# Charrrrrlie/X-as-Supervision

Hardware: AMD Instinct MI355X
Metric: images/sec HM36_Multi_SurS1 256px bs32 (full disc+gen training step) (higher is better)
Workload: dtype f32 (f16x3 split: every fp32 operand as two fp16 pieces, three products; f32 accumulate); 1 GPU; HM36_Multi_SurS1; batch_per_gpu=32, cameras=4, image=256x256, parallelism=dp1, ranks=1, precision=f16x3, dedupe=False, full=False

## Files before the change

include/xas_hip.h:

```cpp
#ifndef XAS_HIP_H
#define XAS_HIP_H

#include <stddef.h>
#include <stdint.h>

#ifdef __cplusplus
extern "C" {
#endif

const char* xas_last_error(void);
enum {
  XAS_TUNE_WGRAD_SPLIT_XCD = 1,
  XAS_TUNE_PLAIN_KLOOP = 32,
  XAS_TUNE_GLOBAL_LOAD = 64,
  XAS_TUNE_WGRAD_GLOBAL_LOAD = 128,
  XAS_TUNE_WGRAD_ALT_ORDER = 8192,
  XAS_TUNE_WGRAD_PLAIN_KLOOP = 524288,
  XAS_TUNE_SLAB_SHIFT = 15,
  XAS_TUNE_SLAB_MASK = 3,
  XAS_TUNE_SLAB_512 = 32768,
  XAS_TUNE_SLAB_128 = 65536,
  XAS_TUNE_SLAB_64 = 98304,
  XAS_TUNE_COL_REDUCE_LEAN = 262144,
  XAS_TUNE_GENERAL_KERNELS = 1 << 22,
// ... 164 lines not shown
int xas_mask_blur_threshold(const uint8_t* mask, int B, int P, uint8_t* out, void* stream);
int xas_patch_finish(const uint8_t* img_bgr, const uint8_t* mask, const float* color_scale, const float* mean3,
                     const float* std3, int rm_bg, int B, int P, float* out_img, float* out_mask, void* stream);
size_t xas_geodesic_workspace_bytes(int B, int P);
int xas_geodesic_weight(const float* mask, const int* centers, const float* params5, int B, int P, float* out,
                        int* center_out, void* workspace, void* stream);
int xas_geodesic_weight_multi(const float* mask, const int* centers, int num_centers, int order, const float* params5, int B, int P,
                              float* out, int* center_out, void* workspace, void* stream);

int xas_loss_nblk(long n);
int xas_mask_loss_fwd(const float* m, const float* gt, const float* weight, long n, int mode,
                      float* partial, float* out, void* stream);
int xas_mask_loss_bwd(const float* m, const float* gt, const float* weight, long n, int mode,
                      const float* out, const float* grad_scalar, float* dm, void* stream);

int xas_pose_loss_fwd(const float* pred, const float* gt, int B, int Hy, int K, int kind, float w0, float w1,
                      float w2, float* out, void* stream);
int xas_pose_loss_bwd(const float* pred, const float* gt, int B, int Hy, int K, int kind, float w0, float w1,
                      float w2, const float* out, const float* grad_scalar, float* grad_pred, float* grad_aux,
                      void* stream);
int xas_lsgan_fwd(const float* logits, int B, int Hy, float target, float* out, int* idx, void* stream);
int xas_lsgan_bwd(const float* logits, int B, int Hy, float target, const int* idx, const float* grad_scalar,
                  float* grad_logits, void* stream);

int xas_graph_aggregate(const float* x, const float* adj, int B, int N, int C, float* y, void* stream);
size_t xas_gln_workspace_floats(long n, int groups, int C);
int xas_gln_fwd(const float* x, const float* gamma, const float* beta, const float* residual,
                long rows, int C, int groups, float eps, float* y, float* stats, float* workspace,
                void* stream);
int xas_gln_bwd(const float* x, const float* beta, const float* dy, const float* gamma,
                const float* stats, long rows, int C, int groups, float eps, float* dx, float* dgamma,
                float* dbeta, float* workspace, void* stream);

int xas_smpl_lbs_fwd(const float* pose , const float* betas ,
                     const float* v_template , const float* shapedirs ,
                     const float* posedirs , const float* j_regressor ,
                     const float* weights , const int* parents , int B, int V,
                     int center_idx, float* verts , float* joints ,
                     float* workspace , void* stream);

size_t xas_smpl_lbs_bwd_workspace_floats(int B, int V);
int xas_smpl_lbs_bwd(const float* pose, const float* betas, const float* v_template, const float* shapedirs,
                     const float* posedirs, const float* j_regressor, const float* weights, const int* parents, int B,
                     int V, int center_idx, const float* fwd_workspace, const float* d_verts, const float* d_joints,
                     float* d_pose, float* d_betas, float* workspace, void* stream);

int xas_adam_step(float* p, const float* g, float* m, float* v, long n, float lr, float beta1,
                  float beta2, float eps, int step, void* stream);


#define XAS_EVAL_CONFIDENT 1
#define XAS_EVAL_SWITCH_ALL 2
#define XAS_EVAL_GT_NORMALISED 4
int xas_eval_select(const float* kps, const float* joints, const int* perm, int B, int Hy, int K, int C,
                    float image_size, int flags, float* sel3d, float* sel2d, float* err2d,
                    unsigned char* swapped, void* stream);

int xas_projection_matrix(const float* k_mat, const float* rot_world, const float* trans_world, int B, float* P,
                          void* stream);

int xas_triangulate_dlt(const float* points, const float* P, int B, int V, int K, float* out, void* stream);

int xas_pose_metrics(const float* pred, const float* gt, const unsigned char* mask, int N, int K, float in_div,
                     int pck_align, float pck_threshold, float* err, float* aligned, float* pck, int* auc_hits,
                     void* stream);

// ... 5 lines not shown
```

x-as-supervision_amd/modules/discriminator.py:

```python
import math

import torch
import torch.nn as nn

from modules.gcn import GCN_SAGE_residual, GCN_residual, GCN_simple
from xas_amd import layers as L


class FFNHeader(nn.Module):
    def __init__(self, in_channels, hidden_channels, p_dropout=0.2):
        super().__init__()
        self.layer1 = L.Linear(in_channels, hidden_channels)
        self.layer2 = L.Linear(hidden_channels, 1)
        self.p = p_dropout
        self.drop_mask = None

    def forward(self, x):
        h = torch.relu(self.layer1(x))
        if self.training and self.p > 0:
            keep = self.drop_mask if self.drop_mask is not None else (torch.rand_like(h) >= self.p).to(h.dtype)
            h = h * keep / (1.0 - self.p)
        return self.layer2(h)


class GCNDiscriminator_base(nn.Module):
    def __init__(self, cfg):
        super().__init__()
        self.input_dim = cfg['input_dim']
        self.hidden_dim = cfg['hidden_dim']
        self.output_dim = cfg['output_dim']
        self.disc_sup_dim = cfg['disc_sup_dim']
        self.num_nodes = cfg['num_node']
        self.use_self_loop = cfg['use_self_loop']
        self.input_layer = nn.Identity()
        self.gcn = nn.Identity()
        self.header = L.Linear(self.output_dim * self.num_nodes, 1)
        self.parent_ids, self.child_ids = None, None
        self._graph_key, self._graph = None, None
# ... 55 lines not shown
            self.num_layers = cfg['num_layers']
            self.gcn = nn.Sequential(
                GCN_simple(self.input_dim, self.hidden_dim, self_loop=sl),
                *[GCN_residual(self.hidden_dim, self.hidden_dim, self.hidden_dim, self_loop=sl, use_bn=cfg['use_bn'])
                  for _ in range(self.num_layers)],
                GCN_simple(self.hidden_dim, self.output_dim, self_loop=sl))
        else:
            raise NotImplementedError
        self.input_layer = L.Linear(self.disc_sup_dim, self.input_dim)

    def compute_graph_matrix(self, keypoints):
        B = keypoints.shape[0]
        pidx, cidx = self._bone_index(keypoints.device)
        diff = keypoints[:, pidx, :] - keypoints[:, cidx, :]
        inv = 1.0 / torch.sqrt(torch.sum(diff ** 2, dim=-1))
        n = self.num_nodes
        w = torch.eye(n, device=keypoints.device).repeat(B, 1, 1) if self.use_self_loop else \
            torch.zeros(B, n, n, device=keypoints.device)
        w = w.index_put((torch.arange(B, device=keypoints.device)[:, None], pidx[None, :], cidx[None, :]), inv)
        w = w.index_put((torch.arange(B, device=keypoints.device)[:, None], cidx[None, :], pidx[None, :]), inv)
        return w

    def forward(self, keypoints):
        B = keypoints.shape[0]
        adj = self.compute_graph_matrix(keypoints)
        x = self.input_layer(keypoints.reshape(B * self.num_nodes, -1))
        return self.header_forward(self.gcn((x, adj))[0], B)

    def forward_groups(self, inputs):
        return [self(x) for x in inputs]


def _stream(hidden, out, num_layers):
    return nn.Sequential(*[GCN_SAGE_residual(hidden, hidden, hidden) for _ in range(num_layers)],
                         GCN_SAGE_residual(hidden, -1, out, single_layer=True))


class GCNSAGEDiscriminator(GCNDiscriminator_base):
    def __init__(self, cfg):
        super().__init__(cfg)
        self.name = 'ResSAGEGCN'
        self.num_layers = cfg['num_layers']
        self.gcn = _stream(self.hidden_dim, self.output_dim, self.num_layers)
        self.use_pe = cfg['use_pe'] if 'use_pe' in cfg else False
        self.input_layer = L.Linear(self.disc_sup_dim * (2 if self.use_pe else 1), self.input_dim)

    def _forward(self, keypoints, groups=1):
        B = keypoints.shape[0]
        g = self.graph(B, keypoints.device) + (groups,)
        if self.use_pe:
            keypoints = torch.cat([keypoints, self.cal_positional_encoding(keypoints)], dim=-1)
        x = self.input_layer(keypoints.reshape(B * self.num_nodes, -1))
        return self.header_forward(self.gcn((x, g))[0], B)


class GCNDiscriminatorDecouple(GCNDiscriminator_base):
    def __init__(self, cfg):
        super().__init__(cfg)
        self.use_pe = cfg['use_pe'] if 'use_pe' in cfg else False
        cin = self.disc_sup_dim * (2 if self.use_pe else 1)
        self.joint_input_layer = L.Linear(cin, self.input_dim)
        self.bone_input_layer = L.Linear(cin, self.input_dim)
        self.name = 'ResGCNDecouple'
        self.num_layers = cfg['num_layers']
        self.joint_gcn = _stream(self.hidden_dim, self.output_dim, self.num_layers)
        self.bone_gcn = _stream(self.hidden_dim, self.output_dim, self.num_layers)
        self.header = FFNHeader(self.output_dim * self.num_nodes * 2, 512)

# ... 19 lines not shown
```

x-as-supervision_amd/modules/gcn.py:

```python
import torch
import torch.nn as nn

from xas_amd import layers as L
from xas_amd import ops_misc


def my_batched_dense_to_sparse(adj):
    if adj.dim() < 2 or adj.dim() > 3:
        raise ValueError(f"Dense adjacency matrix 'adj' must be two- or three-dimensional (got {adj.dim()} dimensions)")
    if adj.dim() == 2:
        idx = adj.nonzero().t()
        return idx, adj[idx[0], idx[1]]
    B, N, M = adj.shape
    flat = adj.reshape(B * N, M)
    idx = flat.nonzero().t().clone()
    vals = flat[idx[0], idx[1]]
    idx[1] += (idx[0] // N) * M
    return idx, vals


class SAGEConv(nn.Module):

    def __init__(self, cin, cout):
        super().__init__()
        self.lin_l = L.Linear(cin, cout, bias=True)
        self.lin_r = L.Linear(cin, cout, bias=False)

    def forward(self, x, graph):
        adj, adj_t, B, N = graph[:4]
        return self.lin_l(ops_misc.graph_aggregate(x, adj, adj_t, B, N)) + self.lin_r(x)


class GraphLayerNorm(nn.Module):
    def __init__(self, c, eps=1e-5):
        super().__init__()
        self.eps = eps
        self.weight = nn.Parameter(torch.ones(c))
        self.bias = nn.Parameter(torch.zeros(c))


class GCN_SAGE_residual(nn.Module):
    def __init__(self, input_dim, hidden_dim, output_dim, single_layer=False):
        super().__init__()
        self.single_layer = single_layer
        if single_layer:
            self.gc1 = SAGEConv(input_dim, output_dim)
            self.ln1 = GraphLayerNorm(output_dim)
            self.gc2 = nn.Identity()
        else:
            self.gc1 = SAGEConv(input_dim, hidden_dim)
            self.ln1 = GraphLayerNorm(hidden_dim)
            self.gc2 = SAGEConv(hidden_dim, output_dim)
            self.ln2 = GraphLayerNorm(output_dim)

    def forward(self, input):
        x, graph = input
        groups = graph[4] if len(graph) > 4 else 1
        y = ops_misc.graph_layernorm_relu(self.gc1(x, graph), self.ln1.weight, self.ln1.bias, None, self.ln1.eps, groups)
        if self.single_layer:
            return (y, graph)
        y = ops_misc.graph_layernorm_relu(self.gc2(y, graph), self.ln2.weight, self.ln2.bias, x, self.ln2.eps, groups)
        return (y, graph)


class GCNConv(nn.Module):

    def __init__(self, cin, cout, add_self_loops=True):
        super().__init__()
        self.lin = L.Linear(cin, cout, bias=False)
        self.bias = nn.Parameter(torch.zeros(cout))
        self.add_self_loops = add_self_loops

    def norm(self, adj):
        if self.add_self_loops:
            diag = adj.diagonal(dim1=1, dim2=2)
            adj = adj + torch.diag_embed((diag == 0).to(adj.dtype))
        deg = adj.sum(dim=1)
        dis = deg.pow(-0.5)
        dis = torch.where(torch.isinf(dis), torch.zeros_like(dis), dis)
        return dis.unsqueeze(2) * adj * dis.unsqueeze(1)

    def forward(self, x, adj):
        B, N = adj.shape[:2]
        xw = self.lin(x).view(B, N, -1)
        out = torch.bmm(self.norm(adj).transpose(1, 2), xw)
        return out.reshape(B * N, -1) + self.bias


class GCN_simple(nn.Module):
    def __init__(self, input_dim, output_dim, self_loop=False):
        super().__init__()
        self.gc = GCNConv(input_dim, output_dim, add_self_loops=self_loop)

    def forward(self, input):
        x, adj = input
# ... 31 lines not shown
```

x-as-supervision_amd/xas_amd/_lib.py:

```python
import ctypes
import os

import torch

_HERE = os.path.dirname(os.path.abspath(__file__))
LIB_PATH = os.environ.get('XAS_HIP_LIB') or os.path.join(_HERE, 'libxas_hip.so')
_lib = None
ABI_VERSION = 3

_T = {'p': ctypes.c_void_p, 'i': ctypes.c_int, 'l': ctypes.c_long, 'f': ctypes.c_float, 'u': ctypes.c_uint,
      'd': ctypes.c_double, 'z': ctypes.c_size_t}


class ConvShape(ctypes.Structure):
    _fields_ = [(n, ctypes.c_int) for n in ('N', 'Hi', 'Wi', 'Cin', 'Cout', 'R', 'S', 'stride', 'pad', 'Ho', 'Wo', 'mode')] + [
        ('grad_amax', ctypes.c_void_p),
        ('x_amax', ctypes.c_void_p)]


PREC_F32, PREC_BF16, PREC_BF16X6, PREC_F16X3 = 0, 1, 2, 3
PREC_NAMES = {'f32': PREC_F32, 'bf16': PREC_BF16, 'bf16x6': PREC_BF16X6, 'f16x3': PREC_F16X3}

TUNE_WGRAD_SPLIT_XCD = 1
TUNE_PLAIN_KLOOP, TUNE_GLOBAL_LOAD, TUNE_WGRAD_GLOBAL_LOAD = 32, 64, 128
# ... 55 lines not shown
    'xas_col_sum_acc': ('plippp', 'i'),
    'xas_bn_apply': ('ppppppfiliippp', 'i'),
    'xas_bn_apply_amax': ('ppppppfiliipppp', 'i'),
    'xas_abs_max': ('plpp', 'i'),
    'xas_bn_update_running': ('ppppfliip', 'i'),
    'xas_bn_bwd_reduce': ('pppppppfiliipppppp', 'i'),
    'xas_bn_bwd_apply': ('ppppppppfiliidpppp', 'i'),
    'xas_bn_bwd_apply_amax': ('ppppppppfiliidppppp', 'i'),
    'xas_maxpool3x3s2_fwd': ('piiiippp', 'i'),
    'xas_maxpool3x3s2_bwd': ('ppiiiipp', 'i'),
    'xas_upsample2x_fwd': ('piiiipp', 'i'),
    'xas_upsample2x_bwd': ('piiiipp', 'i'),
    'xas_sigmoid_fwd': ('plpp', 'i'),
    'xas_sigmoid_bwd': ('pplpp', 'i'),
    'xas_nchw_to_nhwc': ('piiiipp', 'i'),
    'xas_nhwc_to_nchw': ('piiiipp', 'i'),
    'xas_warp_affine_u8': ('ppppiiipp', 'i'),
    'xas_mask_blur_threshold': ('piipp', 'i'),
    'xas_patch_finish': ('pppppiiippp', 'i'),
    'xas_geodesic_workspace_bytes': ('ii', 'z'),
    'xas_geodesic_weight': ('pppiipppp', 'i'),
    'xas_geodesic_weight_multi': ('ppiipiipppp', 'i'),
    'xas_loss_nblk': ('l', 'i'),
    'xas_mask_loss_fwd': ('pppliPpp'.replace('P', 'p'), 'i'),
    'xas_mask_loss_bwd': ('pppliPppp'.replace('P', 'p'), 'i'),
    'xas_pose_loss_fwd': ('ppiiiifffpp', 'i'),
    'xas_pose_loss_bwd': ('ppiiiifffppppp', 'i'),
    'xas_lsgan_fwd': ('piifppp', 'i'),
    'xas_lsgan_bwd': ('piifpppp', 'i'),
    'xas_graph_aggregate': ('ppiiipp', 'i'),
    'xas_gln_workspace_floats': ('lii', 'z'),
    'xas_gln_fwd': ('ppppliifpppp', 'i'),
    'xas_gln_bwd': ('pppppliifppppp', 'i'),
    'xas_smpl_lbs_fwd': ('ppppppppiiipppp', 'i'),
    'xas_smpl_lbs_bwd_workspace_floats': ('ii', 'z'),
    'xas_smpl_lbs_bwd': ('ppppppppiiippppppp', 'i'),
    'xas_adam_step': ('pppplffffip', 'i'),
    'xas_eval_select': ('pppiiiifippppp', 'i'),
    'xas_projection_matrix': ('pppipp', 'i'),
    'xas_triangulate_dlt': ('ppiiipp', 'i'),
    'xas_pose_metrics': ('pppiififppppp', 'i'),
}


def load():
    global _lib
    if _lib is not None:
        return _lib
    if not os.path.exists(LIB_PATH):
        raise RuntimeError('libxas_hip.so is missing (%s): run `python __graft_entry__.py` to build the HIP '
                           'library; the MI355X path has no CPU fallback' % LIB_PATH)
    lib = ctypes.CDLL(LIB_PATH)
    lib.xas_abi_version.restype = ctypes.c_int
    lib.xas_abi_version.argtypes = []
    if lib.xas_abi_version() != ABI_VERSION:
        raise RuntimeError('%s speaks ABI version %d, this binding expects %d (include/xas_hip.h): rebuild it with '
                           '`python __graft_entry__.py`' % (LIB_PATH, lib.xas_abi_version(), ABI_VERSION))
    lib.xas_last_error.restype = ctypes.c_char_p
    lib.xas_last_error.argtypes = []
    _lib = lib
    mode = os.environ.get('XAS_PRECISION', '')
    if mode != '':
        lib.xas_set_precision.argtypes = [ctypes.c_int]
        lib.xas_set_precision.restype = ctypes.c_int
        if lib.xas_set_precision(int(mode)) != 0:
            raise RuntimeError('XAS_PRECISION=%s: %s' % (mode, lib.xas_last_error().decode()))
# ... 49 lines not shown
```

x-as-supervision_amd/xas_amd/ops_misc.py:

```python
import torch

from ._lib import call, ptr, query


class _MaskLoss(torch.autograd.Function):
    @staticmethod
    def forward(ctx, m, gt, weight, use_clip):
        m, gt = m.contiguous(), gt.contiguous()
        w = weight.contiguous() if weight is not None else None
        n = m.numel()
        mode = (1 if use_clip else 0) | (2 if w is not None else 0)
        partial = torch.empty(query('xas_loss_nblk', n) * 2, device=m.device, dtype=torch.float32)
        out = torch.empty(3, device=m.device, dtype=torch.float32)
        call('xas_mask_loss_fwd', ptr(m), ptr(gt), ptr(w), n, mode, ptr(partial), ptr(out))
        ctx.save_for_backward(m, gt, w if w is not None else m.new_empty(0), out)
        ctx.mode = mode
        return out[2]

    @staticmethod
    def backward(ctx, g):
        m, gt, w, out = ctx.saved_tensors
        dm = torch.empty_like(m)
        call('xas_mask_loss_bwd', ptr(m), ptr(gt), ptr(w) if ctx.mode & 2 else None, m.numel(), ctx.mode, ptr(out),
             ptr(g.contiguous().reshape(1)), ptr(dm))
        return dm, None, None, None


def mask_loss(mask, gt, weight=None, use_clip=False):
    return _MaskLoss.apply(mask, gt, weight, use_clip)


class _GraphAggregate(torch.autograd.Function):
    @staticmethod
    def forward(ctx, x, adj, adj_t, B, N):
# ... 21 lines not shown

class _GraphLayerNormRelu(torch.autograd.Function):
    @staticmethod
    def forward(ctx, x, gamma, beta, residual, eps, groups):
        x = x.contiguous()
        rows_all, C = x.shape
        rows = rows_all // groups
        y = torch.empty_like(x)
        stats = torch.empty(groups * 2, device=x.device, dtype=torch.float32)
        ws = torch.empty(query('xas_gln_workspace_floats', rows * C, groups, C), device=x.device, dtype=torch.float32)
        res = residual.contiguous() if residual is not None else None
        call('xas_gln_fwd', ptr(x), ptr(gamma), ptr(beta), ptr(res), rows, C, groups, float(eps), ptr(y), ptr(stats), ptr(ws))
        ctx.save_for_backward(x, gamma, beta, stats)
        ctx.cfg = (float(eps), residual is not None, groups, rows)
        return y

    @staticmethod
    def backward(ctx, dy):
        x, gamma, beta, stats = ctx.saved_tensors
        eps, has_res, groups, rows = ctx.cfg
        C = x.shape[1]
        dy = dy.contiguous()
        dx = torch.empty_like(x)
        dg = torch.empty_like(gamma)
        db = torch.empty_like(beta)
        ws = torch.empty(query('xas_gln_workspace_floats', rows * C, groups, C), device=x.device, dtype=torch.float32)
        call('xas_gln_bwd', ptr(x), ptr(beta), ptr(dy), ptr(gamma), ptr(stats), rows, C, groups, eps, ptr(dx), ptr(dg),
             ptr(db), ptr(ws))
        return dx, dg, db, (dy if has_res else None), None, None


def graph_layernorm_relu(x, gamma, beta, residual=None, eps=1e-5, groups=1):
    return _GraphLayerNormRelu.apply(x, gamma, beta, residual, eps, groups)


class _SmplLbs(torch.autograd.Function):

    @staticmethod
    def forward(ctx, pose, betas, v_template, shapedirs, posedirs, j_regressor, weights, parents, center_idx):
        B, V = pose.shape[0], v_template.shape[-2]
        dev = pose.device
        pose, betas = pose.contiguous(), betas.contiguous()
        bufs = tuple(t.contiguous() for t in (v_template, shapedirs, posedirs, j_regressor, weights))
        verts = torch.empty(B, V, 3, device=dev, dtype=torch.float32)
        joints = torch.empty(B, 24, 3, device=dev, dtype=torch.float32)
        ws = torch.empty(B * (72 + 24 * 16 + 207), device=dev, dtype=torch.float32)
        c = -1 if center_idx is None else int(center_idx)
        call('xas_smpl_lbs_fwd', ptr(pose), ptr(betas), *(ptr(t) for t in bufs), ptr(parents), B, V, c, ptr(verts),
             ptr(joints), ptr(ws))
        ctx.save_for_backward(pose, betas, *bufs, parents, ws)
        ctx.cfg = (B, V, c)
        return verts, joints

    @staticmethod
    def backward(ctx, d_verts, d_joints):
        pose, betas, vt, sd, pd, jr, w, parents, ws = ctx.saved_tensors
        B, V, c = ctx.cfg
        d_pose, d_betas = torch.empty_like(pose), torch.empty_like(betas)
        dv = d_verts.contiguous() if d_verts is not None else torch.zeros(B, V, 3, device=pose.device)
        dj = d_joints.contiguous() if d_joints is not None else None
        ws2 = torch.empty(query('xas_smpl_lbs_bwd_workspace_floats', B, V), device=pose.device, dtype=torch.float32)
        call('xas_smpl_lbs_bwd', ptr(pose), ptr(betas), ptr(vt), ptr(sd), ptr(pd), ptr(jr), ptr(w), ptr(parents), B, V, c,
             ptr(ws), ptr(dv), ptr(dj), ptr(d_pose), ptr(d_betas), ptr(ws2))
        return d_pose, d_betas, None, None, None, None, None, None, None


# ... 61 lines not shown
```

Before: 2078 images/s.

## Fuse GraphSAGE residual stack into tiled MFMA kernels with inline layernorm

Adds a fused HIP path for stacks of SAGEConv + graph layernorm + ReLU + residual layers in the discriminator. Each forward kernel applies the previous layer's layernorm and ReLU, does the adjacency aggregation in shared memory, and runs both linear projections with fp32 MFMA. It also emits per-tile partial statistics so the next layer can normalise without a separate pass. The backward pass has fused data and parameter-gradient kernels that write gradients straight into existing .grad buffers. This replaces many small launches and intermediate tensors, but adds a large amount of custom code and shape restrictions (C≤128, N≤18).

```diff
diff --git a/include/xas_hip.h b/include/xas_hip.h
--- a/include/xas_hip.h
+++ b/include/xas_hip.h
@@ -220,6 +220,28 @@
                 const float* stats, long rows, int C, int groups, float eps, float* dx, float* dgamma,
                 float* dbeta, float* workspace, void* stream);
 
+int xas_sage_tile_samples(void);
+int xas_sage_tiles(int B, int groups);
+int xas_sage_fwd(const float* zin, const float* part_in, const float* gamma, const float* beta,
+                 const float* res, float* h_out, float* stats_out, const float* adj, const float* wl,
+                 const float* bl, const float* wr, int B, int N, int C, int groups, float eps, float* z,
+                 float* part_out, void* stream);
+int xas_sage_ln_apply(const float* z, const float* part, const float* gamma, const float* beta,
+                      const float* res, int B, int N, int C, int groups, float eps, float* h,
+                      float* stats, void* stream);
+int xas_sage_ln_bwd_sums(const float* g, const float* z, const float* stats, const float* gamma,
+                         const float* beta, int B, int N, int C, int groups, float eps, float* psum,
+                         void* stream);
+int xas_sage_bwd_data(const float* g, const float* z, const float* stats, const float* psum,
+                      const float* gamma, const float* beta, const float* wl, const float* wr,
+                      const float* adj_t, const float* gres, const float* z_below,
+                      const float* stats_below, const float* gamma_below, const float* beta_below,
+                      int B, int N, int C, int groups, float eps, float eps_below, float* dz,
+                      float* g_below, float* psum_below, void* stream);
+int xas_sage_bwd_params(const float* dz, const float* h, const float* adj, const float* psum, int B,
+                        int N, int C, int groups, float* gwl, float* gbl, float* gwr, float* ggamma,
+                        float* gbeta, void* stream);
+
 int xas_smpl_lbs_fwd(const float* pose , const float* betas ,
                      const float* v_template , const float* shapedirs ,
                      const float* posedirs , const float* j_regressor ,
diff --git a/x-as-supervision_amd/csrc/gcn.hip b/x-as-supervision_amd/csrc/gcn.hip
--- /dev/null
+++ b/x-as-supervision_amd/csrc/gcn.hip
@@ -0,0 +1,562 @@
+#include "common.h"
+
+namespace xas {
+
+typedef float f32x16 __attribute__((ext_vector_type(16)));
+
+constexpr int kSageT = 3;
+constexpr int kSageMaxN = 18;
+constexpr int kSageMaxC = 128;
+constexpr int kSageRows = kSageT * kSageMaxN;
+constexpr int kSageLD = kSageMaxC + 4;
+
+__device__ __forceinline__ float gln_xhat(float x, float mean, float inv) { return __fmul_rn(__fsub_rn(x, mean), inv); }
+__device__ __forceinline__ float gln_pre(float xh, float g, float b) { return __fmaf_rn(xh, g, b); }
+
+struct SageTile {
+  int g, ti, R;
+  long row0;
+};
+__device__ __forceinline__ SageTile sage_tile(int B, int N, int tpg) {
+  SageTile t;
+  t.g = blockIdx.x / tpg;
+  t.ti = blockIdx.x % tpg;
+  const int s0 = t.ti * kSageT;
+  const int ns = (B - s0 < kSageT) ? B - s0 : kSageT;
+  t.R = ns * N;
+  t.row0 = ((long)t.g * B + s0) * N;
+  return t;
+}
+
+__device__ __forceinline__ void sage_group_stats(const float* __restrict__ part, int g, int tpg, float* out) {
+  const int lane = threadIdx.x & 63;
+  const float* pg = part + (size_t)g * tpg * 4;
+  const double P = (double)pg[0];
+  double a = 0.0, b = 0.0, n = 0.0;
+  for (int i = lane; i < tpg; i += 64) {
+    const double d = (double)pg[i * 4] - P, cnt = (double)pg[i * 4 + 1], s1 = (double)pg[i * 4 + 2], s2 = (double)pg[i * 4 + 3];
+    a += s1 + cnt * d;
+    b += s2 + 2.0 * d * s1 + cnt * d * d;
+    n += cnt;
+  }
+#pragma unroll
+  for (int o = 32; o > 0; o >>= 1) {
+    a += __shfl_xor(a, o, 64);
+    b += __shfl_xor(b, o, 64);
+    n += __shfl_xor(n, o, 64);
+  }
+  if (lane == 0) {
+    const double m = a / n;
+    double v = b / n - m * m;
+    if (v < 0.0) v = 0.0;
+    out[0] = (float)(P + m);
+    out[1] = (float)sqrt(v);
+  }
+}
+
+__device__ __forceinline__ f32x16 zero16() {
+  f32x16 v;
+#pragma unroll
+  for (int e = 0; e < 16; ++e) v[e] = 0.f;
+  return v;
+}
+
+__device__ __forceinline__ int mfma_row(int reg, int half) { return (reg & 3) + 8 * (reg >> 2) + 4 * half; }
+
+struct SageFwdArgs {
+  const float* zin;
+  const float* part_in;
+  const float* gamma;
+  const float* beta;
+  const float* res;
+  float* h_out;
+  float* stats_out;
+  const float* adj;
+  const float* wl;
+  const float* bl;
+  const float* wr;
+  float* z;
+  float* part_out;
+  int B, N, C, tpg;
+  float eps;
+};
+
+__global__ __launch_bounds__(256) void sage_fwd_kernel(SageFwdArgs a) {
+  __shared__ __attribute__((aligned(16))) float hs[kSageRows * kSageLD];
+  __shared__ __attribute__((aligned(16))) float ags[kSageRows * kSageLD];
+  __shared__ float adj_s[kSageMaxN * kSageMaxN];
+  __shared__ float st[2];
+  __shared__ float red[20];
+  __shared__ float s_piv;
+  const SageTile t = sage_tile(a.B, a.N, a.tpg);
+  const int C = a.C, N = a.N, R = t.R, C4 = C >> 2;
+  const int tid = threadIdx.x, lane = tid & 63, wave = tid >> 6;
+  for (int e = tid; e < N * N; e += 256) adj_s[e] = a.adj[e];
+  if (a.part_in && tid < 64) sage_group_stats(a.part_in, t.g, a.tpg, st);
+  __syncthreads();
+  float mean = 0.f, inv = 0.f;
+  if (a.part_in) {
+    mean = st[0];
+    inv = 1.f / (st[1] + a.eps);
+    if (t.ti == 0 && tid == 0) { a.stats_out[t.g * 2] = st[0]; a.stats_out[t.g * 2 + 1] = st[1]; }
+  }
+  for (int e = tid; e < R * C4; e += 256) {
+    const int r = e / C4, c = (e % C4) * 4;
+    const size_t off = (size_t)(t.row0 + r) * C + c;
+    float4 v = *reinterpret_cast<const float4*>(a.zin + off);
+    if (a.part_in) {
+      const float4 g4 = *reinterpret_cast<const float4*>(a.gamma + c), b4 = *reinterpret_cast<const float4*>(a.beta + c);
+      v.x = fmaxf(gln_pre(gln_xhat(v.x, mean, inv), g4.x, b4.x), 0.f);
+      v.y = fmaxf(gln_pre(gln_xhat(v.y, mean, inv), g4.y, b4.y), 0.f);
+      v.z = fmaxf(gln_pre(gln_xhat(v.z, mean, inv), g4.z, b4.z), 0.f);
+      v.w = fmaxf(gln_pre(gln_xhat(v.w, mean, inv), g4.w, b4.w), 0.f);
+      if (a.res) {
+        const float4 r4 = *reinterpret_cast<const float4*>(a.res + off);
+        v.x += r4.x; v.y += r4.y; v.z += r4.z; v.w += r4.w;
+      }
+      *reinterpret_cast<float4*>(a.h_out + off) = v;
+    }
+    *reinterpret_cast<float4*>(&hs[r * kSageLD + c]) = v;
+  }
+  __syncthreads();
+  for (int e = tid; e < R * C4; e += 256) {
+    const int r = e / C4, c = (e % C4) * 4;
+    const int node = r % N, sb = r - node;
+    float4 acc = make_float4(0.f, 0.f, 0.f, 0.f);
+    for (int j = 0; j < N; ++j) {
+      const float w = adj_s[node * N + j];
+      if (w != 0.f) {
+        const float4 x4 = *reinterpret_cast<const float4*>(&hs[(sb + j) * kSageLD + c]);
+        acc.x = fmaf(w, x4.x, acc.x); acc.y = fmaf(w, x4.y, acc.y); acc.z = fmaf(w, x4.z, acc.z); acc.w = fmaf(w, x4.w, acc.w);
+      }
+    }
+    *reinterpret_cast<float4*>(&ags[r * kSageLD + c]) = acc;
+  }
+  __syncthreads();
+  const int j = lane & 31, hh = lane >> 5, n0 = wave * 32;
+  const int nmb = (R + 31) >> 5;
+  f32x16 acc[2];
+  float sa = 0.f, sb2 = 0.f;
+  if (n0 < C) {
+    const float bias = a.bl[n0 + j];
+#pragma unroll
+    for (int e = 0; e < 16; ++e) { acc[0][e] = bias; acc[1][e] = bias; }
+    const int r0 = (j < R) ? j : R - 1, r1 = (32 + j < R) ? 32 + j : R - 1;
+#pragma unroll
+    for (int ph = 0; ph < 2; ++ph) {
+      const float* A = ph ? hs : ags;
+      const float* W = (ph ? a.wr : a.wl) + (size_t)(n0 + j) * C + 4 * hh;
+      const float* A0 = A + r0 * kSageLD + 4 * hh;
+      const float* A1 = A + r1 * kSageLD + 4 * hh;
+
+      for (int q = 0; q < C; q += 8) {
+        const float4 b4 = *reinterpret_cast<const float4*>(W + q);
+        const float4 a0 = *reinterpret_cast<const float4*>(A0 + q);
+        acc[0] = __builtin_amdgcn_mfma_f32_32x32x2f32(a0.x, b4.x, acc[0], 0, 0, 0);
+        acc[0] = __builtin_amdgcn_mfma_f32_32x32x2f32(a0.y, b4.y, acc[0], 0, 0, 0);
+        acc[0] = __builtin_amdgcn_mfma_f32_32x32x2f32(a0.z, b4.z, acc[0], 0, 0, 0);
+        acc[0] = __builtin_amdgcn_mfma_f32_32x32x2f32(a0.w, b4.w, acc[0], 0, 0, 0);
+        if (nmb > 1) {
+          const float4 a1 = *reinterpret_cast<const float4*>(A1 + q);
+          acc[1] = __builtin_amdgcn_mfma_f32_32x32x2f32(a1.x, b4.x, acc[1], 0, 0, 0);
+          acc[1] = __builtin_amdgcn_mfma_f32_32x32x2f32(a1.y, b4.y, acc[1], 0, 0, 0);
+          acc[1] = __builtin_amdgcn_mfma_f32_32x32x2f32(a1.z, b4.z, acc[1], 0, 0, 0);
+          acc[1] = __builtin_amdgcn_mfma_f32_32x32x2f32(a1.w, b4.w, acc[1], 0, 0, 0);
+        }
+      }
+    }
+    if (wave == 0 && lane == 0) s_piv = acc[0][0];
+  }
+  __syncthreads();
+  if (n0 < C) {
+    const float piv = s_piv;
+#pragma unroll
+    for (int mb = 0; mb < 2; ++mb) {
+#pragma unroll
+      for (int reg = 0; reg < 16; ++reg) {
+        const int row = mb * 32 + mfma_row(reg, hh);
+        if (row < R) {
+          const float v = acc[mb][reg];
+          a.z[(size_t)(t.row0 + row) * C + n0 + j] = v;
+          const float d = v - piv;
+          sa += d;
+          sb2 = fmaf(d, d, sb2);
+        }
+      }
+    }
+  }
+  sa = block_sum(sa, red);
+  sb2 = block_sum(sb2, red);
+  if (tid == 0) {
+    float* o = a.part_out + (size_t)blockIdx.x * 4;
+    o[0] = s_piv; o[1] = (float)(R * C); o[2] = sa; o[3] = sb2;
+  }
+}
+
+__global__ __launch_bounds__(256) void sage_ln_apply_kernel(const float* __restrict__ z, const float* __restrict__ part,
+                                                            const float* __restrict__ gamma, const float* __restrict__ beta,
+                                                            const float* __restrict__ res, int B, int N, int C, int tpg,
+                                                            float eps, float* __restrict__ h, float* __restrict__ stats) {
+  __shared__ float st[2];
+  const SageTile t = sage_tile(B, N, tpg);
+  const int tid = threadIdx.x, C4 = C >> 2;
+  if (tid < 64) sage_group_stats(part, t.g, tpg, st);
+  __syncthreads();
+  const float mean = st[0], inv = 1.f / (st[1] + eps);
+  if (t.ti == 0 && tid == 0) { stats[t.g * 2] = st[0]; stats[t.g * 2 + 1] = st[1]; }
+  for (int e = tid; e < t.R * C4; e += 256) {
+    const int r = e / C4, c = (e % C4) * 4;
+    const size_t off = (size_t)(t.row0 + r) * C + c;
+    float4 v = *reinterpret_cast<const float4*>(z + off);
+    const float4 g4 = *reinterpret_cast<const float4*>(gamma + c), b4 = *reinterpret_cast<const float4*>(beta + c);
+    v.x = fmaxf(gln_pre(gln_xhat(v.x, mean, inv), g4.x, b4.x), 0.f);
+    v.y = fmaxf(gln_pre(gln_xhat(v.y, mean, inv), g4.y, b4.y), 0.f);
+    v.z = fmaxf(gln_pre(gln_xhat(v.z, mean, inv), g4.z, b4.z), 0.f);
+    v.w = fmaxf(gln_pre(gln_xhat(v.w, mean, inv), g4.w, b4.w), 0.f);
+    if (res) {
+      const float4 r4 = *reinterpret_cast<const float4*>(res + off);
+      v.x += r4.x; v.y += r4.y; v.z += r4.z; v.w += r4.w;
+    }
+    *reinterpret_cast<float4*>(h + off) = v;
+  }
+}
+
+__device__ __forceinline__ void sage_tile_ln_sums(const float* G, int ldg, const float* __restrict__ z,
+                                                  const float* __restrict__ stats, const float* __restrict__ gamma,
+                                                  const float* __restrict__ beta, const SageTile& t, int C, float eps,
+                                                  float* __restrict__ psum) {
+  const int c = threadIdx.x;
+  if (c >= C) return;
+  const float mean = stats[t.g * 2], inv = 1.f / (stats[t.g * 2 + 1] + eps);
+  const float gm = gamma[c], bt = beta[c];
+  const float* zp = z + (size_t)t.row0 * C + c;
+  float s1 = 0.f, s2 = 0.f;
+  for (int r = 0; r < t.R; ++r) {
+    const float xh = gln_xhat(zp[(size_t)r * C], mean, inv);
+    const float gg = (gln_pre(xh, gm, bt) > 0.f) ? G[(size_t)r * ldg + c] : 0.f;
+    s1 += gg;
+    s2 = fmaf(gg, xh, s2);
+  }
+  psum[((size_t)blockIdx.x * 2) * C + c] = s1;
+  psum[((size_t)blockIdx.x * 2 + 1) * C + c] = s2;
+}
+
+__global__ __launch_bounds__(256) void sage_ln_bwd_sums_kernel(const float* __restrict__ G, const float* __restrict__ z,
+                                                               const float* __restrict__ stats,
+                                                               const float* __restrict__ gamma, const float* __restrict__ beta,
+                                                               int B, int N, int C, int tpg, float eps,
+                                                               float* __restrict__ psum) {
+  const SageTile t = sage_tile(B, N, tpg);
+  sage_tile_ln_sums(G + (size_t)t.row0 * C, C, z, stats, gamma, beta, t, C, eps, psum);
+}
+
+struct SageBwdArgs {
+  const float* G;
+  const float* z;
+  const float* stats;
+  const float* psum;
+  const float* gamma;
+  const float* beta;
+  const float* wl;
+  const float* wr;
+  const float* adj_t;
+  const float* gres;
+  const float* z_below;
+  const float* stats_below;
+  const float* gamma_below;
+  const float* beta_below;
+  float* dz;
+  float* g_below;
+  float* psum_below;
+  int B, N, C, tpg;
+  float eps, eps_below;
+};
+
+__global__ __launch_bounds__(256) void sage_bwd_data_kernel(SageBwdArgs a) {
+  __shared__ __attribute__((aligned(16))) float dzs[kSageRows * kSageLD];
+  __shared__ __attribute__((aligned(16))) float us[kSageRows * kSageLD];
+  __shared__ float adj_s[kSageMaxN * kSageMaxN];
+  __shared__ float red[20];
+  const SageTile t = sage_tile(a.B, a.N, a.tpg);
+  const int C = a.C, N = a.N, R = t.R, C4 = C >> 2;
+  const int tid = threadIdx.x, lane = tid & 63, wave = tid >> 6;
+  for (int e = tid; e < N * N; e += 256) adj_s[e] = a.adj_t[e];
+  float sa = 0.f, sb = 0.f;
+  if (tid < C) {
+    double s1 = 0.0, s2 = 0.0;
+    for (int i = 0; i < a.tpg; ++i) {
+      const float* p = a.psum + ((size_t)(t.g * a.tpg + i) * 2) * C;
+      s1 += (double)p[tid];
+      s2 += (double)p[C + tid];
+    }
+    sa = a.gamma[tid] * (float)s1;
+    sb = a.gamma[tid] * (float)s2;
+  }
+  sa = block_sum(sa, red);
+  sb = block_sum(sb, red);
+  const float mean = a.stats[t.g * 2], sigma = a.stats[t.g * 2 + 1], inv = 1.f / (sigma + a.eps);
+  const float n = (float)((long)a.B * N * C);
+  const float A = sa / n, Bc = sigma > 0.f ? sb / (n * sigma) : 0.f;
+  for (int e = tid; e < R * C4; e += 256) {
+    const int r = e / C4, c = (e % C4) * 4;
+    const size_t off = (size_t)(t.row0 + r) * C + c;
+    const float4 g4 = *reinterpret_cast<const float4*>(a.G + off), z4 = *reinterpret_cast<const float4*>(a.z + off);
+    const float4 gm = *reinterpret_cast<const float4*>(a.gamma + c), bt = *reinterpret_cast<const float4*>(a.beta + c);
+    float4 d;
+    float xh;
+    xh = gln_xhat(z4.x, mean, inv); d.x = ((gln_pre(xh, gm.x, bt.x) > 0.f ? g4.x * gm.x : 0.f) - A) * inv - xh * Bc;
+    xh = gln_xhat(z4.y, mean, inv); d.y = ((gln_pre(xh, gm.y, bt.y) > 0.f ? g4.y * gm.y : 0.f) - A) * inv - xh * Bc;
+    xh = gln_xhat(z4.z, mean, inv); d.z = ((gln_pre(xh, gm.z, bt.z) > 0.f ? g4.z * gm.z : 0.f) - A) * inv - xh * Bc;
+    xh = gln_xhat(z4.w, mean, inv); d.w = ((gln_pre(xh, gm.w, bt.w) > 0.f ? g4.w * gm.w : 0.f) - A) * inv - xh * Bc;
+    *reinterpret_cast<float4*>(a.dz + off) = d;
+    *reinterpret_cast<float4*>(&dzs[r * kSageLD + c]) = d;
+  }
+  __syncthreads();
+  const int j = lane & 31, hh = lane >> 5, i0 = wave * 32;
+  const int nmb = (R + 31) >> 5;
+  f32x16 au[2], av[2];
+  au[0] = zero16(); au[1] = zero16(); av[0] = zero16(); av[1] = zero16();
+  if (i0 < C) {
+    const int r0 = (j < R) ? j : R - 1, r1 = (32 + j < R) ? 32 + j : R - 1;
+    const float* A0 = dzs + r0 * kSageLD + 4 * hh;
+    const float* A1 = dzs + r1 * kSageLD + 4 * hh;
+    const float* WL = a.wl + (size_t)(4 * hh) * C + i0 + j;
+    const float* WR = a.wr + (size_t)(4 * hh) * C + i0 + j;
+
+    for (int q = 0; q < C; q += 8) {
+      float bl[4], br[4];
+#pragma unroll
+      for (int s = 0; s < 4; ++s) { bl[s] = WL[(size_t)(q + s) * C]; br[s] = WR[(size_t)(q + s) * C]; }
+      const float4 a0 = *reinterpret_cast<const float4*>(A0 + q);
+      const float a0v[4] = {a0.x, a0.y, a0.z, a0.w};
+#pragma unroll
+      for (int s = 0; s < 4; ++s) {
+        au[0] = __builtin_amdgcn_mfma_f32_32x32x2f32(a0v[s], bl[s], au[0], 0, 0, 0);
+        av[0] = __builtin_amdgcn_mfma_f32_32x32x2f32(a0v[s], br[s], av[0], 0, 0, 0);
+      }
+      if (nmb > 1) {
+        const float4 a1 = *reinterpret_cast<const float4*>(A1 + q);
+        const float a1v[4] = {a1.x, a1.y, a1.z, a1.w};
+#pragma unroll
+        for (int s = 0; s < 4; ++s) {
+          au[1] = __builtin_amdgcn_mfma_f32_32x32x2f32(a1v[s], bl[s], au[1], 0, 0, 0);
+          av[1] = __builtin_amdgcn_mfma_f32_32x32x2f32(a1v[s], br[s], av[1], 0, 0, 0);
+        }
+      }
+    }
+#pragma unroll
+    for (int mb = 0; mb < 2; ++mb) {
+#pragma unroll
+      for (int reg = 0; reg < 16; ++reg) {
+        const int row = mb * 32 + mfma_row(reg, hh);
+        if (row < R) us[row * kSageLD + i0 + j] = au[mb][reg];
+      }
+    }
+  }
+  __syncthreads();
+  if (i0 < C) {
+#pragma unroll
+    for (int mb = 0; mb < 2; ++mb) {
+#pragma unroll
+      for (int reg = 0; reg < 16; ++reg) {
+        const int row = mb * 32 + mfma_row(reg, hh);
+        if (row < R) {
+          const int node = row % N, sb0 = row - node;
+          float v = av[mb][reg];
+          for (int k = 0; k < N; ++k) {
+            const float w = adj_s[node * N + k];
+            if (w != 0.f) v = fmaf(w, us[(sb0 + k) * kSageLD + i0 + j], v);
+          }
+          const size_t off = (size_t)(t.row0 + row) * C + i0 + j;
+          if (a.gres) v += a.gres[off];
+          a.g_below[off] = v;
+          dzs[row * kSageLD + i0 + j] = v;
+        }
+      }
+    }
+  }
+  __syncthreads();
+  if (a.z_below)
+    sage_tile_ln_sums(dzs, kSageLD, a.z_below, a.stats_below, a.gamma_below, a.beta_below, t, C, a.eps_below, a.psum_below);
+}
+
+__global__ __launch_bounds__(1024) void sage_bwd_params_kernel(const float* __restrict__ dz, const float* __restrict__ h,
+                                                               const float* __restrict__ adj, const float* __restrict__ psum,
+                                                               int S, int N, int C, int ntiles, float* __restrict__ gwl,
+                                                               float* __restrict__ gbl, float* __restrict__ gwr,
+                                                               float* __restrict__ ggamma, float* __restrict__ gbeta) {
+  __shared__ float red[8 * 16 * 64];
+  __shared__ float adj_s[kSageMaxN * kSageMaxN];
+  const int tid = threadIdx.x, lane = tid & 63, wave = tid >> 6;
+  const int nb = C >> 5;
+  const int bid = blockIdx.x;
+  if (bid < 2 * nb * nb) {
+    const int which = bid / (nb * nb), ob = (bid / nb) % nb, ib = bid % nb;
+    const int j = lane & 31, hh = lane >> 5;
+    for (int e = tid; e < N * N; e += 1024) adj_s[e] = adj[e];
+    __syncthreads();
+    f32x16 acc = zero16();
+    const int np = (N + 1) >> 1;
+    for (int s = wave; s < S; s += 16) {
+      const float* hp = h + (size_t)s * N * C + ib * 32 + j;
+      const float* dp = dz + (size_t)s * N * C + ob * 32 + j;
+      if (which) {
+        for (int p = 0; p < np; ++p) {
+          const int r = 2 * p + hh;
+          const float av = (r < N) ? dp[(size_t)r * C] : 0.f;
+          const float bv = (r < N) ? hp[(size_t)r * C] : 0.f;
+          acc = __builtin_amdgcn_mfma_f32_32x32x2f32(av, bv, acc, 0, 0, 0);
+        }
+      } else {
+        float hc[kSageMaxN];
+#pragma unroll
+        for (int k = 0; k < kSageMaxN; ++k) hc[k] = (k < N) ? hp[(size_t)k * C] : 0.f;
+        for (int p = 0; p < np; ++p) {
+          const int r = 2 * p + hh;
+          const float av = (r < N) ? dp[(size_t)r * C] : 0.f;
+          float bv = 0.f;
+          if (r < N) {
+#pragma unroll
+            for (int k = 0; k < kSageMaxN; ++k)
+              if (k < N) bv = fmaf(adj_s[r * N + k], hc[k], bv);
+          }
+          acc = __builtin_amdgcn_mfma_f32_32x32x2f32(av, bv, acc, 0, 0, 0);
+        }
+      }
+    }
+    for (int half = 8; half >= 1; half >>= 1) {
+      if (wave >= half && wave < 2 * half) {
+#pragma unroll
+        for (int reg = 0; reg < 16; ++reg) red[((wave - half) * 16 + reg) * 64 + lane] = acc[reg];
+      }
+      __syncthreads();
+      if (wave < half) {
+#pragma unroll
+        for (int reg = 0; reg < 16; ++reg) acc[reg] += red[(wave * 16 + reg) * 64 + lane];
+      }
+      __syncthreads();
+    }
+    if (wave == 0) {
+      float* gw = which ? gwr : gwl;
+#pragma unroll
+      for (int reg = 0; reg < 16; ++reg) {
+        const int o = ob * 32 + mfma_row(reg, hh);
+        gw[(size_t)o * C + ib * 32 + j] += acc[reg];
+      }
+    }
+  } else {
+    const int cx = tid & 31, ry = tid >> 5;
+    const int col = (bid - 2 * nb * nb) * 32 + cx;
+    const long rows = (long)S * N;
+    float a0 = 0.f, a1 = 0.f, a2 = 0.f, a3 = 0.f;
+    for (long r = ry; r < rows; r += 128) {
+      a0 += dz[(size_t)r * C + col];
+      if (r + 32 < rows) a1 += dz[(size_t)(r + 32) * C + col];
+      if (r + 64 < rows) a2 += dz[(size_t)(r + 64) * C + col];
+      if (r + 96 < rows) a3 += dz[(size_t)(r + 96) * C + col];
+    }
+    float s1 = 0.f, s2 = 0.f;
+    for (int t = ry; t < ntiles; t += 32) {
+      s1 += psum[((size_t)t * 2) * C + col];
+      s2 += psum[((size_t)t * 2 + 1) * C + col];
+    }
+    red[(0 * 32 + ry) * 32 + cx] = (a0 + a1) + (a2 + a3);
+    red[(1 * 32 + ry) * 32 + cx] = s1;
+    red[(2 * 32 + ry) * 32 + cx] = s2;
+    __syncthreads();
+    if (ry == 0) {
+      float u = 0.f, v = 0.f, w = 0.f;
+      for (int k = 0; k < 32; ++k) { u += red[k * 32 + cx]; v += red[(32 + k) * 32 + cx]; w += red[(64 + k) * 32 + cx]; }
+      gbl[col] += u;
+      gbeta[col] += v;
+      ggamma[col] += w;
+    }
+  }
+}
+
+static bool sage_dims_ok(int B, int N, int C, int groups) {
+  return B > 0 && groups > 0 && N > 0 && N <= kSageMaxN && C > 0 && C <= kSageMaxC && C % 32 == 0 &&
+         (long)groups * cdiv(B, kSageT) < (1L << 30);
+}
+static bool aligned16(const void* p) { return (reinterpret_cast<uintptr_t>(p) & 15) == 0; }
+
+}
+
+using namespace xas;
+
+#define SAGE_DIMS_MSG "sage: needs 1 <= N <= 18, C a multiple of 32 up to 128, B >= 1, groups >= 1"
+
+extern "C" int xas_sage_tile_samples(void) { return kSageT; }
+
+extern "C" int xas_sage_tiles(int B, int groups) {
+  if (B <= 0 || groups <= 0) return 0;
+  return (int)(groups * cdiv(B, kSageT));
+}
+
+extern "C" int xas_sage_fwd(const float* zin, const float* part_in, const float* gamma, const float* beta, const float* res,
+                            float* h_out, float* stats_out, const float* adj, const float* wl, const float* bl,
+                            const float* wr, int B, int N, int C, int groups, float eps, float* z, float* part_out,
+                            void* stream) {
+  XAS_REQUIRE(sage_dims_ok(B, N, C, groups), SAGE_DIMS_MSG);
+  XAS_REQUIRE(zin && adj && wl && bl && wr && z && part_out, "sage_fwd: null buffer");
+  XAS_REQUIRE(!part_in || (gamma && beta && h_out && stats_out), "sage_fwd: the LayerNorm on load needs gamma, beta, h_out and stats_out");
+  XAS_REQUIRE(aligned16(zin) && aligned16(gamma) && aligned16(beta) && aligned16(res) && aligned16(h_out) && aligned16(wl) &&
+                  aligned16(wr) && aligned16(z), "sage_fwd: buffers must be 16-byte aligned");
+  SageFwdArgs a{zin, part_in, gamma, beta, res, h_out, stats_out, adj, wl, bl, wr, z, part_out, B, N, C, (int)cdiv(B, kSageT), eps};
+  hipLaunchKernelGGL(sage_fwd_kernel, dim3((unsigned)xas_sage_tiles(B, groups)), dim3(256), 0, as_stream(stream), a);
+  XAS_LAUNCH_CHECK();
+  return 0;
+}
+
+extern "C" int xas_sage_ln_apply(const float* z, const float* part, const float* gamma, const float* beta, const float* res,
+                                 int B, int N, int C, int groups, float eps, float* h, float* stats, void* stream) {
+  XAS_REQUIRE(sage_dims_ok(B, N, C, groups), SAGE_DIMS_MSG);
+  XAS_REQUIRE(z && part && gamma && beta && h && stats, "sage_ln_apply: null buffer");
+  XAS_REQUIRE(aligned16(z) && aligned16(gamma) && aligned16(beta) && aligned16(res) && aligned16(h),
+              "sage_ln_apply: buffers must be 16-byte aligned");
+  hipLaunchKernelGGL(sage_ln_apply_kernel, dim3((unsigned)xas_sage_tiles(B, groups)), dim3(256), 0, as_stream(stream), z, part,
+                     gamma, beta, res, B, N, C, (int)cdiv(B, kSageT), eps, h, stats);
+  XAS_LAUNCH_CHECK();
+  return 0;
+}
+
+extern "C" int xas_sage_ln_bwd_sums(const float* g, const float* z, const float* stats, const float* gamma, const float* beta,
+                                    int B, int N, int C, int groups, float eps, float* psum, void* stream) {
+  XAS_REQUIRE(sage_dims_ok(B, N, C, groups), SAGE_DIMS_MSG);
+  XAS_REQUIRE(g && z && stats && gamma && beta && psum, "sage_ln_bwd_sums: null buffer");
+  hipLaunchKernelGGL(sage_ln_bwd_sums_kernel, dim3((unsigned)xas_sage_tiles(B, groups)), dim3(256), 0, as_stream(stream), g, z,
+                     stats, gamma, beta, B, N, C, (int)cdiv(B, kSageT), eps, psum);
+  XAS_LAUNCH_CHECK();
+  return 0;
+}
+
+extern "C" int xas_sage_bwd_data(const float* g, const float* z, const float* stats, const float* psum, const float* gamma,
+                                 const float* beta, const float* wl, const float* wr, const float* adj_t, const float* gres,
+                                 const float* z_below, const float* stats_below, const float* gamma_below,
+                                 const float* beta_below, int B, int N, int C, int groups, float eps, float eps_below,
+                                 float* dz, float* g_below, float* psum_below, void* stream) {
+  XAS_REQUIRE(sage_dims_ok(B, N, C, groups), SAGE_DIMS_MSG);
+  XAS_REQUIRE(g && z && stats && psum && gamma && beta && wl && wr && adj_t && dz && g_below, "sage_bwd_data: null buffer");
+  XAS_REQUIRE(!z_below || (stats_below && gamma_below && beta_below && psum_below),
+              "sage_bwd_data: the sums of the layer below need its stats, gamma, beta and psum_below");
+  XAS_REQUIRE(aligned16(g) && aligned16(z) && aligned16(gamma) && aligned16(beta) && aligned16(dz),
+              "sage_bwd_data: buffers must be 16-byte aligned");
+  SageBwdArgs a{g, z, stats, psum, gamma, beta, wl, wr, adj_t, gres, z_below, stats_below, gamma_below, beta_below,
+                dz, g_below, psum_below, B, N, C, (int)cdiv(B, kSageT), eps, eps_below};
+  hipLaunchKernelGGL(sage_bwd_data_kernel, dim3((unsigned)xas_sage_tiles(B, groups)), dim3(256), 0, as_stream(stream), a);
+  XAS_LAUNCH_CHECK();
+  return 0;
+}
+
+extern "C" int xas_sage_bwd_params(const float* dz, const float* h, const float* adj, const float* psum, int B, int N, int C,
+                                   int groups, float* gwl, float* gbl, float* gwr, float* ggamma, float* gbeta,
+                                   void* stream) {
+  XAS_REQUIRE(sage_dims_ok(B, N, C, groups), SAGE_DIMS_MSG);
+  XAS_REQUIRE(dz && h && adj && psum && gwl && gbl && gwr && ggamma && gbeta, "sage_bwd_params: null buffer");
+  XAS_REQUIRE((long)B * groups < (1L << 24), "sage_bwd_params: too many samples");
+  const int nb = C / 32;
+  hipLaunchKernelGGL(sage_bwd_params_kernel, dim3((unsigned)(2 * nb * nb + nb)), dim3(1024), 0, as_stream(stream), dz, h, adj,
+                     psum, B * groups, N, C, xas_sage_tiles(B, groups), gwl, gbl, gwr, ggamma, gbeta);
+  XAS_LAUNCH_CHECK();
+  return 0;
+}
diff --git a/x-as-supervision_amd/modules/discriminator.py b/x-as-supervision_amd/modules/discriminator.py
--- a/x-as-supervision_amd/modules/discriminator.py
+++ b/x-as-supervision_amd/modules/discriminator.py
@@ -3,7 +3,7 @@
 import torch
 import torch.nn as nn
 
-from modules.gcn import GCN_SAGE_residual, GCN_residual, GCN_simple
+from modules.gcn import GCN_SAGE_residual, GCN_residual, GCN_simple, SAGEStream
 from xas_amd import layers as L
 
 
@@ -125,8 +125,8 @@
 
 
 def _stream(hidden, out, num_layers):
-    return nn.Sequential(*[GCN_SAGE_residual(hidden, hidden, hidden) for _ in range(num_layers)],
-                         GCN_SAGE_residual(hidden, -1, out, single_layer=True))
+    return SAGEStream(*[GCN_SAGE_residual(hidden, hidden, hidden) for _ in range(num_layers)],
+                      GCN_SAGE_residual(hidden, -1, out, single_layer=True))
 
 
 class GCNSAGEDiscriminator(GCNDiscriminator_base):
diff --git a/x-as-supervision_amd/modules/gcn.py b/x-as-supervision_amd/modules/gcn.py
--- a/x-as-supervision_amd/modules/gcn.py
+++ b/x-as-supervision_amd/modules/gcn.py
@@ -53,14 +53,45 @@
             self.gc2 = SAGEConv(hidden_dim, output_dim)
             self.ln2 = GraphLayerNorm(output_dim)
 
+    def sage_layers(self, first):
+        def entry(gc, ln, res):
+            return ((gc.lin_l.weight, gc.lin_l.bias, gc.lin_r.weight, ln.weight, ln.bias), res, ln.eps)
+        if self.single_layer:
+            return [entry(self.gc1, self.ln1, -1)]
+        return [entry(self.gc1, self.ln1, -1), entry(self.gc2, self.ln2, first)]
+
     def forward(self, input):
         x, graph = input
+        y = sage_blocks_fused([self], x, graph)
+        if y is not None:
+            return (y, graph)
         groups = graph[4] if len(graph) > 4 else 1
         y = ops_misc.graph_layernorm_relu(self.gc1(x, graph), self.ln1.weight, self.ln1.bias, None, self.ln1.eps, groups)
         if self.single_layer:
             return (y, graph)
         y = ops_misc.graph_layernorm_relu(self.gc2(y, graph), self.ln2.weight, self.ln2.bias, x, self.ln2.eps, groups)
         return (y, graph)
+
+
+def sage_blocks_fused(blocks, x, graph):
+    adj, adj_t, B, N = graph[:4]
+    groups = graph[4] if len(graph) > 4 else 1
+    layers = []
+    for blk in blocks:
+        layers += blk.sage_layers(len(layers))
+    if B % groups or x.shape[0] != B * N or not ops_misc.sage_fusable(x, N, layers):
+        return None
+    return ops_misc.sage_stack(x, adj, adj_t, B // groups, N, groups, layers)
+
+
+class SAGEStream(nn.Sequential):
+
+    def forward(self, input):
+        x, graph = input
+        y = sage_blocks_fused(list(self), x, graph)
+        if y is not None:
+            return (y, graph)
+        return super().forward(input)
 
 
 class GCNConv(nn.Module):
diff --git a/x-as-supervision_amd/xas_amd/_lib.py b/x-as-supervision_amd/xas_amd/_lib.py
--- a/x-as-supervision_amd/xas_amd/_lib.py
+++ b/x-as-supervision_amd/xas_amd/_lib.py
@@ -111,6 +111,13 @@
     'xas_gln_workspace_floats': ('lii', 'z'),
     'xas_gln_fwd': ('ppppliifpppp', 'i'),
     'xas_gln_bwd': ('pppppliifppppp', 'i'),
+    'xas_sage_tile_samples': ('', 'i'),
+    'xas_sage_tiles': ('ii', 'i'),
+    'xas_sage_fwd': ('ppppppppppp' 'iiii' 'f' 'ppp', 'i'),
+    'xas_sage_ln_apply': ('ppppp' 'iiii' 'f' 'ppp', 'i'),
+    'xas_sage_ln_bwd_sums': ('ppppp' 'iiii' 'f' 'pp', 'i'),
+    'xas_sage_bwd_data': ('pppppppppppppp' 'iiii' 'ff' 'pppp', 'i'),
+    'xas_sage_bwd_params': ('pppp' 'iiii' 'pppppp', 'i'),
     'xas_smpl_lbs_fwd': ('ppppppppiiipppp', 'i'),
     'xas_smpl_lbs_bwd_workspace_floats': ('ii', 'z'),
     'xas_smpl_lbs_bwd': ('ppppppppiiippppppp', 'i'),
diff --git a/x-as-supervision_amd/xas_amd/ops_misc.py b/x-as-supervision_amd/xas_amd/ops_misc.py
--- a/x-as-supervision_amd/xas_amd/ops_misc.py
+++ b/x-as-supervision_amd/xas_amd/ops_misc.py
@@ -1,5 +1,8 @@
+import os
+
 import torch
 
+from . import ops_nn
 from ._lib import call, ptr, query
 
 
@@ -87,6 +90,117 @@
 
 def graph_layernorm_relu(x, gamma, beta, residual=None, eps=1e-5, groups=1):
     return _GraphLayerNormRelu.apply(x, gamma, beta, residual, eps, groups)
+
+
+DISC_FUSED = os.environ.get('XAS_DISC_FUSED', '1') == '1'
+SAGE_MAX_C, SAGE_MAX_N = 128, 18
+
+
+def sage_fusable(x, N, layers):
+    if not (DISC_FUSED and x.is_cuda and x.dtype == torch.float32 and x.dim() == 2 and 0 < N <= SAGE_MAX_N):
+        return False
+    C = x.shape[1]
+    if C % 32 or C > SAGE_MAX_C or x.shape[0] == 0:
+        return False
+    for ps, _res, _eps in layers:
+        wl, bl, wr, gm, bt = ps
+        if tuple(wl.shape) != (C, C) or tuple(wr.shape) != (C, C) or bl is None:
+            return False
+        if any(p.dtype != torch.float32 or not p.is_cuda or not p.is_contiguous() or p.data_ptr() % 16 for p in ps):
+            return False
+    return True
+
+
+def _grad_target(p, need, like):
+    if not need:
+        return torch.zeros_like(like), None, None
+    g = p.grad if (p is not None and p.is_leaf) else None
+    if g is not None and g.is_cuda and g.dtype == torch.float32 and g.is_contiguous() and g.shape == like.shape:
+        return g, None, p
+    t = torch.zeros_like(like)
+    return t, t, None
+
+
+class _SageStack(torch.autograd.Function):
+
+    @staticmethod
+    def forward(ctx, x, adj, adj_t, B, N, groups, cfg, plist, *params):
+        x = x.contiguous()
+        C, L = x.shape[1], len(cfg)
+        dev = x.device
+        tiles = query('xas_sage_tiles', B, groups)
+        new = lambda *s: torch.empty(*s, device=dev, dtype=torch.float32)
+        hs, zs, parts, stats = [x], [], [], []
+        for k in range(L):
+            wl, bl, wr = params[5 * k:5 * k + 3]
+            z, part = torch.empty_like(x), new(tiles * 4)
+            if k == 0:
+                call('xas_sage_fwd', ptr(x), None, None, None, None, None, None, ptr(adj), ptr(wl), ptr(bl), ptr(wr), B, N, C,
+                     groups, 0.0, ptr(z), ptr(part))
+            else:
+                r, eps = cfg[k - 1]
+                h, st = torch.empty_like(x), new(groups * 2)
+                call('xas_sage_fwd', ptr(zs[-1]), ptr(parts[-1]), ptr(params[5 * k - 2]), ptr(params[5 * k - 1]),
+                     ptr(hs[r]) if r >= 0 else None, ptr(h), ptr(st), ptr(adj), ptr(wl), ptr(bl), ptr(wr), B, N, C, groups,
+                     float(eps), ptr(z), ptr(part))
+                hs.append(h)
+                stats.append(st)
+            zs.append(z)
+            parts.append(part)
+        r, eps = cfg[L - 1]
+        h, st = torch.empty_like(x), new(groups * 2)
+        call('xas_sage_ln_apply', ptr(zs[-1]), ptr(parts[-1]), ptr(params[5 * L - 2]), ptr(params[5 * L - 1]),
+             ptr(hs[r]) if r >= 0 else None, B, N, C, groups, float(eps), ptr(h), ptr(st))
+        stats.append(st)
+        ctx.save_for_backward(adj, adj_t, *hs, *zs, *stats, *params)
+        ctx.cfg, ctx.dims, ctx.plist, ctx.tiles = cfg, (B, N, C, groups, L), plist, tiles
+        return h
+
+    @staticmethod
+    def backward(ctx, dh):
+        B, N, C, groups, L = ctx.dims
+        cfg, tiles = ctx.cfg, ctx.tiles
+        sv = ctx.saved_tensors
+        adj, adj_t = sv[0], sv[1]
+        hs, zs, stats, params = sv[2:2 + L], sv[2 + L:2 + 2 * L], sv[2 + 2 * L:2 + 3 * L], sv[2 + 3 * L:]
+        dev = dh.device
+        new = lambda *s: torch.empty(*s, device=dev, dtype=torch.float32)
+        G = {L: dh.contiguous()}
+        psum = new(tiles * 2 * C)
+        call('xas_sage_ln_bwd_sums', ptr(G[L]), ptr(zs[L - 1]), ptr(stats[L - 1]), ptr(params[5 * L - 2]),
+             ptr(params[5 * L - 1]), B, N, C, groups, float(cfg[L - 1][1]), ptr(psum))
+        dz = torch.empty_like(G[L])
+        grads = [None] * (5 * L)
+        for k in range(L, 0, -1):
+            wl, bl, wr, gm, bt = params[5 * k - 5:5 * k]
+            takers = [m for m in range(1, L + 1) if cfg[m - 1][0] == k - 1]
+            assert len(takers) <= 1 and all(m >= k for m in takers)
+            gres = G[takers[0]] if takers else None
+            gb = torch.empty_like(dz)
+            below = k >= 2
+            psb = new(tiles * 2 * C) if below else None
+            call('xas_sage_bwd_data', ptr(G[k]), ptr(zs[k - 1]), ptr(stats[k - 1]), ptr(psum), ptr(gm), ptr(bt), ptr(wl), ptr(wr),
+                 ptr(adj_t), ptr(gres), ptr(zs[k - 2]) if below else None, ptr(stats[k - 2]) if below else None,
+                 ptr(params[5 * k - 7]) if below else None, ptr(params[5 * k - 6]) if below else None, B, N, C, groups,
+                 float(cfg[k - 1][1]), float(cfg[k - 2][1]) if below else 0.0, ptr(dz), ptr(gb), ptr(psb))
+            need = ctx.needs_input_grad[8 + 5 * k - 5:8 + 5 * k]
+            if any(need):
+                tg = [_grad_target(p, n, t) for p, n, t in zip(ctx.plist[5 * k - 5:5 * k], need, (wl, bl, wr, gm, bt))]
+                call('xas_sage_bwd_params', ptr(dz), ptr(hs[k - 1]), ptr(adj), ptr(psum), B, N, C, groups,
+                     *(ptr(t[0]) for t in tg))
+                for i, (_buf, ret, p) in enumerate(tg):
+                    grads[5 * k - 5 + i] = ret
+                    if p is not None:
+                        ops_nn.grad_ready(p)
+            G[k - 1] = gb
+            psum = psb
+        return (G[0], None, None, None, None, None, None, None, *grads)
+
+
+def sage_stack(x, adj, adj_t, B, N, groups, layers):
+    cfg = tuple((int(r), float(e)) for _ps, r, e in layers)
+    plist = [p for ps, _r, _e in layers for p in ps]
+    return _SageStack.apply(x, adj, adj_t, B, N, groups, cfg, plist, *plist)
 
 
 class _SmplLbs(torch.autograd.Function):
```

After: 2025 images/s. 0.974x the previous value.
